# vgl-hub/kreeq

Hardware: AMD Instinct MI355X
Metric: distinct+total k-mers/sec at k=21 (count path) (higher is better)
Workload: dtype u64

## Files before the change

kreeq_amd/csrc/kq_kernels.h:

```cpp
#pragma once

#include <hip/hip_runtime.h>

#include <type_traits>

#include "../../include/kreeq_amd.h"
#include "kq_device.h"
#include "kq_partition.h"

using namespace kq;


__global__ __launch_bounds__(TILE_THREADS) void k_count_direct(TableView t, const uint8_t* __restrict__ ab,
                                                                uint64_t lead, uint64_t len, int k, EmitRange er, PartCfg filt,
                                                                const uint16_t* __restrict__ pinv ) {
    uint32_t n_new = 0;
    uint64_t n_kmers = 0;
    scan_tiles(ab, lead, len, k, [&](uint64_t pos, uint64_t fw, uint64_t rv, uint32_t prev, uint32_t next) {
        if (pos < er.lo || pos >= er.hi) return;
        const bool is_fw = fw < rv;
        const uint64_t key = is_fw ? fw : rv;
        if (filt.filt_lo != 0 || filt.filt_hi != filt.map_count) {
            const uint32_t m = map_index(key, filt.map_count, filt.map_mask);
            if (m < filt.filt_lo || m >= filt.filt_hi) return;
// ... 206 lines not shown
        tile_lane_scan_all(s_codes[half], s_inv[half], lo_valid, tile, k, er, [&](int i, bool valid, uint64_t fw, uint64_t rv, uint32_t prev, uint32_t next) {
            const bool is_fw = fw < rv;
            const uint64_t key = is_fw ? fw : rv;
            const uint64_t h = table_hash(key, (uint32_t)k);
            const uint32_t b = valid ? p1_bin_of<BINMODE>(cfg, key, h) : NB;
            if (b != NB) atomicAdd(&s_hist[b], 1u);
            if (TOP8) { s_buf[i * TILE_THREADS + lane] = top8_rec(h, edge_idx6_any(is_fw, prev, next)); s_bin[i * TILE_THREADS + lane] = (uint16_t)b; }
            else s_buf[half * MS_TILE + i * TILE_THREADS + lane] = narrow_word(narrow_main(h), narrow_aux(h, edge_idx6_any(is_fw, prev, next)), b);
        }, lane);
        __syncthreads();
        const uint32_t cnt = bin_owner ? s_hist[tid] : 0u;
        uint32_t incl = cnt;
        if (bin_owner) {
#pragma unroll
            for (int o = 1; o < 64; o <<= 1) { const uint32_t n = __shfl_up(incl, o, 64); if ((tid & 63) >= o) incl += n; }
            if ((tid & 63) == 63) s_wave[tid >> 6] = incl;
        }
        uint64_t w[16];
        uint32_t wb[TOP8 ? 16 : 1];
#pragma unroll
        for (int it = 0; it < 16; ++it) { w[it] = s_buf[half * MS_TILE + it * TILE_THREADS + lane]; if (TOP8) wb[it] = s_bin[it * TILE_THREADS + lane]; }
        __syncthreads();
        if (bin_owner) {
            uint32_t excl = incl - cnt;
            for (int v = 0; v < (tid >> 6); ++v) excl += s_wave[v];
            s_loff[tid] = excl;
            if (tid == (int)NB - 1) s_loff[NB] = excl + cnt;
            s_hist[tid] = excl;
            s_grel[tid] = gabs - excl;
            gabs += cnt;
        }
        __syncthreads();
        uint32_t pl[16];
#pragma unroll
        for (int it = 0; it < 16; ++it) { const uint32_t b = TOP8 ? wb[TOP8 ? it : 0] : narrow_word_bin(w[it]); pl[it] = b != NB ? atomicAdd(&s_hist[b], 1u) : ~0u; }
#pragma unroll
        for (int it = 0; it < 16; ++it) if (pl[it] != ~0u) { s_buf[pl[it]] = w[it]; if (TOP8) s_bin[pl[it]] = (uint16_t)wb[TOP8 ? it : 0]; }
        __syncthreads();
        const uint32_t total = s_loff[NB];
        uint64_t cv[16];
        uint32_t cg[16];
#pragma unroll
        for (int it = 0; it < 16; ++it) cv[it] = s_buf[tid + it * THREADS];
#pragma unroll
        for (int it = 0; it < 16; ++it) cg[it] = s_grel[(uint32_t)(tid + it * THREADS) < total ? (TOP8 ? (uint32_t)s_bin[TOP8 ? tid + it * THREADS : 0] : narrow_word_bin(cv[it])) : 0u] + (tid + it * THREADS);
        if (bin_owner) s_hist[tid] = 0;
        landed(nxt.x); landed(nxt.y); landed(nxt.z); landed(nxt.w);
#pragma unroll
        for (int it = 0; it < 16; ++it) {
            if ((uint32_t)(tid + it * THREADS) < total) {
                if (TOP8) reinterpret_cast<uint64_t*>(recs)[cg[it]] = cv[it];
                else { recs[cg[it]] = (uint32_t)cv[it]; recs_aux[cg[it]] = (uint8_t)(cv[it] >> 48); }
            }
        }
    }
}

__global__ __launch_bounds__(1024) void k_lv_units(const unsigned long long* __restrict__ seg_off, const unsigned long long* __restrict__ seg_hi, LevelCfg lv,
                                                   unsigned long long* __restrict__ unit_base) {
    __shared__ unsigned long long s_part[1024];
    const uint32_t tid = threadIdx.x, per = (lv.n_seg + 1023) / 1024;
    const uint32_t lo = min(tid * per, lv.n_seg), hi = min(lo + per, lv.n_seg);
    unsigned long long sum = 0;
    for (uint32_t b = lo; b < hi; ++b) sum += (seg_hi[b] - seg_off[b] + P2_UNIT - 1) / P2_UNIT;
    s_part[tid] = sum;
    __syncthreads();
    if (tid < 64) {
        unsigned long long loc[16], tot = 0;
#pragma unroll
        for (int j = 0; j < 16; ++j) { loc[j] = s_part[tid * 16 + j]; tot += loc[j]; }
        unsigned long long incl = tot;
#pragma unroll
        for (int o = 1; o < 64; o <<= 1) { unsigned long long nn = __shfl_up(incl, o, 64); if ((int)tid >= o) incl += nn; }
        unsigned long long run = incl - tot;
#pragma unroll
        for (int j = 0; j < 16; ++j) { s_part[tid * 16 + j] = run; run += loc[j]; }
        if (tid == 63) unit_base[lv.n_seg] = incl;
    }
    __syncthreads();
    unsigned long long run = s_part[tid];
    for (uint32_t b = lo; b < hi; ++b) { unit_base[b] = run; run += (seg_hi[b] - seg_off[b] + P2_UNIT - 1) / P2_UNIT; }
}
__device__ __forceinline__ uint32_t seg_of_unit(const unsigned long long* unit_base, uint32_t n_seg, uint64_t u) {
    uint32_t lo = 0, hi = n_seg;
    while (hi - lo > 1) { uint32_t mid = (lo + hi) >> 1; if (unit_base[mid] <= u) lo = mid; else hi = mid; }
    return lo;
}
template <int FMT>
__global__ __launch_bounds__(MS_THREADS) void k_lv_hist(const uint64_t* __restrict__ recs, const uint8_t* __restrict__ , LevelCfg lv,
                                                        const unsigned long long* __restrict__ seg_off, const unsigned long long* __restrict__ seg_hi,
                                                        const unsigned long long* __restrict__ unit_base, uint32_t* __restrict__ m2) {
    __shared__ uint32_t s_hist[NB_MAX];
    const uint64_t n_units = unit_base[lv.n_seg];
    for (uint64_t u = blockIdx.x; u < n_units; u += gridDim.x) {
        const uint32_t b_in = seg_of_unit(unit_base, lv.n_seg, u);
        const uint32_t b = lv.spb > 1 ? b_in / lv.spb : b_in;
        const uint64_t lo = seg_off[b_in] + (u - unit_base[b_in]) * P2_UNIT;
        const uint64_t hi = lo + P2_UNIT < seg_hi[b_in] ? lo + P2_UNIT : seg_hi[b_in];
        for (uint32_t i = threadIdx.x; i < lv.nb; i += MS_THREADS) s_hist[i] = 0;
        __syncthreads();
        const uint64_t last = hi - 1;
        if (FMT == FMT_NARROW) {
            const uint4* v4 = reinterpret_cast<const uint4*>(recs);
            const uint64_t q0 = lo >> 2, q1 = (hi + 3) >> 2;
            for (uint64_t qb = q0; qb < q1; qb += 4ull * MS_THREADS) {
                uint4 q[4];
// ... 1237 lines not shown
```

kreeq_amd/csrc/kreeq_amd.hip:

```cpp
#include <hip/hip_runtime.h>
#include <hipcub/hipcub.hpp>

#include <algorithm>
#include <cstdarg>
#include <cstdio>
#include <cstdlib>
#include <cstring>
#include <mutex>
#include <new>
#include <numeric>
#include <string>
#include <thread>
#include <type_traits>
#include <vector>

#include "../../include/kreeq_amd.h"
#include "kq_device.h"
#include "kq_partition.h"

using namespace kq;

#include "kq_kernels.h"
#include "kq_fastx.h"

// ... 577 lines not shown
    HIPC(hipStreamSynchronize(h->stream));
    std::string out;
    for (size_t i = 1; i < h->marks.size(); ++i) {
        float ms = 0;
        HIPC(hipEventElapsedTime(&ms, h->marks[i - 1].second, h->marks[i].second));
        char tmp[96];
        snprintf(tmp, sizeof tmp, "%s%s=%.4f", out.empty() ? "" : ";", h->marks[i].first, ms);
        out += tmp;
    }
    if (out.size() + 1 > cap) return fail(KQ_ERR_CAPACITY, "profile buffer too small: need %zu", out.size() + 1);
    memcpy(buf, out.c_str(), out.size() + 1);
    return KQ_OK;
}
void* kq_get_stream(kq_handle* h) { return h ? (void*)h->stream : nullptr; }
int kq_sync(kq_handle* h) {
    if (!h) return fail(KQ_ERR_INVALID, "null handle");
    HIPC(hipSetDevice(h->device));
    HIPC(hipStreamSynchronize(h->stream));
    const int rc = check_errors(h);
    if (h->fx_bad) return fail(KQ_ERR_INVALID, "malformed %s text was submitted for counting and skipped (kq_clear resets this)", h->fx_bad == KQ_FASTX_FASTQ ? "FASTQ" : "FASTA");
    return rc;
}
int kq_flush(kq_handle* h) {
    if (!h) return fail(KQ_ERR_INVALID, "null handle");
    HIPC(hipSetDevice(h->device));
    return flush_pending(h);
}
int kq_get_info(kq_handle* h, kq_info* out) {
    if (!h || !out) return fail(KQ_ERR_INVALID, "null argument");
    HIPC(hipSetDevice(h->device));
    int rc = read_state(h);
    if (rc) return rc;
    out->kmers_counted = h->st_host->kmers_added;
    out->slots_used = h->st_host->slots_used;
    out->slots_total = h->n_slots();
    out->hc_used = h->st_host->hc_used;
    out->hc_total = h->hc_cap;
    out->table_bytes = h->n_slots() * sizeof(Slot) + h->hc_cap * sizeof(HcSlot);
    out->table_passes = h->table_passes;
    return KQ_OK;
}

struct PartPlan {
    PartCfg cfg;
    bool two_level;
    int fmt;
    uint64_t n_max, R;
    uint32_t g1;
    uint64_t m1_n, m2_n, sums_n, groups_n;
    uint64_t *recs1, *recs2;
    uint8_t *aux1, *aux2;
    unsigned long long *m1, *seg_off, *unit_base, *group_base, *sums, *total, *hot;
    uint32_t* m2;
};
static void plan_cfg(const kq_handle* h, PartCfg* cfg, bool allow_narrow = false) {
    cfg->n_regions = h->n_regions;
    uint32_t g = 1;
    while (((cfg->n_regions + (1ull << g) - 1) >> g) > 512 && g < 10) ++g;
    while (((cfg->n_regions + (1ull << g) - 1) >> g) >= (uint64_t)NB_MAX) ++g;
    cfg->g_shift = cfg->n_regions < (uint64_t)NB_MAX ? 0 : g;
    cfg->n_coarse = (uint32_t)((cfg->n_regions + (1ull << cfg->g_shift) - 1) >> cfg->g_shift);
    cfg->mode = 0; cfg->map_count = (uint32_t)h->map_count;
    cfg->map_mask = (h->map_count & (h->map_count - 1)) == 0 ? (uint32_t)h->map_count - 1 : 0;
    cfg->filt_lo = 0; cfg->filt_hi = (uint32_t)h->map_count;
    cfg->raw_out = 0;
    cfg->narrow = 0; cfg->sub_bits = 0; cfg->owner_sub = 0; cfg->n_rng = 0; cfg->win_lo = 0; cfg->win_hi = 1u << NARROW_CBITS;
    if (allow_narrow && (h->k <= (int)NARROW_MAX_K || h->k > PART_MAX_K) && cfg->n_regions >= (uint64_t)NB_MAX && cfg->n_regions % (1u << NARROW_CBITS) == 0) {
        const uint64_t rps = cfg->n_regions >> NARROW_CBITS;
        uint32_t sb = 0;
        if (rps >= h->mid_rps) {
            const uint64_t target_nb = std::max<uint64_t>(1, std::min<uint64_t>(256, h->mid_rps / 8));
            while ((rps >> sb) > target_nb && sb < SUB_BITS_MAX && rps % (2ull << sb) == 0) ++sb;
        }
        if ((rps >> sb) < (uint64_t)NB_MAX && (sb > 0 || rps < (uint64_t)NB_MAX)) { cfg->narrow = 1; cfg->sub_bits = sb; }
    }
    if (cfg->narrow) { cfg->n_coarse = 1u << NARROW_CBITS; if (cfg->g_shift == 0) cfg->g_shift = 1; }
}
static int plan_alloc(kq_handle* h, PartPlan* p, uint64_t n_max, uint64_t n_tiles, uint32_t p1_bins, bool allow_narrow = false,
                      uint64_t min_segs = 0 ) {
    if (h->test_fail_plan) { h->test_fail_plan = false; return fail(KQ_ERR_NOMEM, "partition scratch allocation failed (injected by KQ_OPT_TEST_FAIL_PLAN)"); }
    if (n_max >= (1ull << 32) - 16) return fail(KQ_ERR_INVALID, "a partition pass handles fewer than 2^32 records (got %llu): slice the input", (unsigned long long)n_max);
    plan_cfg(h, &p->cfg, allow_narrow);
    n_max = (n_max + 7) & ~7ull;
    p->two_level = p->cfg.g_shift != 0;
    p->fmt = !p->cfg.narrow ? FMT_PACK8 : h->k > PART_MAX_K ? FMT_TOP8 : FMT_NARROW;
    p->n_max = n_max; p->R = p->cfg.n_regions;
    p->g1 = (uint32_t)std::max<uint64_t>(1, std::min<uint64_t>(n_tiles, (uint64_t)h->n_cu * (p1_bins < 512 ? 18 : 12)));
    p->m1_n = (uint64_t)p1_bins * p->g1 * P1_F;
    const uint64_t nb_max = std::max<uint64_t>(std::max<uint64_t>(1ull << p->cfg.g_shift, p->cfg.n_coarse), p->cfg.narrow ? (p->cfg.n_regions >> NARROW_CBITS) >> p->cfg.sub_bits : 0);
    const uint64_t seg_max = std::max<uint64_t>(min_segs, p->cfg.narrow ? ((uint64_t)1 << NARROW_CBITS) << p->cfg.sub_bits : (uint64_t)NB_MAX);
    p->m2_n = (n_max / P2_UNIT + seg_max + 2) * nb_max;
    p->groups_n = std::max<uint64_t>(std::max<uint64_t>(p->R, (uint64_t)p->cfg.n_coarse << p->cfg.g_shift), min_segs) + 2;
    p->sums_n = std::max(p->m1_n, p->groups_n) / SCAN_CHUNK + 2;
    const uint64_t aux_words = (n_max + 7) / 8 + 1;
    const uint64_t rec_words = p->fmt == FMT_NARROW ? n_max / 2 + 2 : n_max;
    const bool split2 = (rec_words + aux_words) * 8 >= ((size_t)512 << 20);
    if (split2) { int rc2 = scr_ensure(h->part2, (size_t)(rec_words + aux_words) * 8, h->device); if (rc2) return rc2; }
    const size_t words = (size_t)((split2 ? 1 : 2) * (rec_words + aux_words) + p->m1_n + 2 * (seg_max + 2) + p->groups_n + p->sums_n + 4 + (p->R + 2) + (p->m2_n + 1) / 2);
    int rc = ensure_buf(&h->part, &h->part_bytes, words * 8);
    if (rc) return rc;
    p->recs1 = (uint64_t*)h->part;
    p->aux1 = (uint8_t*)(p->recs1 + rec_words);
    uint64_t* rest = (uint64_t*)(p->aux1 + aux_words * 8);
    if (split2) { p->recs2 = (uint64_t*)h->part2.p; p->aux2 = (uint8_t*)(p->recs2 + rec_words); }
    else { p->recs2 = rest; p->aux2 = (uint8_t*)(p->recs2 + rec_words); rest = (uint64_t*)(p->aux2 + aux_words * 8); }
    p->m1 = (unsigned long long*)rest;
    p->seg_off = p->m1 + p->m1_n;
    p->unit_base = p->seg_off + seg_max + 2;
    p->group_base = p->unit_base + seg_max + 2;
    p->sums = p->group_base + p->groups_n;
    p->total = p->sums + p->sums_n;
    p->hot = p->total + 4;
    p->m2 = (uint32_t*)(p->hot + p->R + 2);
    return KQ_OK;
}
static void scan_u64(kq_handle* h, unsigned long long* a, uint64_t n, unsigned long long* sums_scratch, unsigned long long* total) {
    if (n <= 2 * SCAN_CHUNK) {
        hipLaunchKernelGGL(k_exclusive_scan, dim3(1), dim3(1024), 0, h->stream, a, n, total);
        return;
    }
    const uint64_t chunks = (n + SCAN_CHUNK - 1) / SCAN_CHUNK;
    hipLaunchKernelGGL(k_scan_sums, dim3((unsigned)chunks), dim3(1024), 0, h->stream, a, n, sums_scratch);
    hipLaunchKernelGGL(k_exclusive_scan, dim3(1), dim3(1024), 0, h->stream, sums_scratch, chunks, total);
    hipLaunchKernelGGL(k_scan_apply, dim3((unsigned)chunks), dim3(1024), 0, h->stream, a, n, sums_scratch);
}
static void mark(kq_handle* h, const char* name) {
    if (!h->profile) return;
    hipEvent_t e;
    if (hipEventCreate(&e) != hipSuccess) return;
    (void)hipEventRecord(e, h->stream);
    h->marks.emplace_back(name, e);
}
static void marks_reset(kq_handle* h) {
    for (auto& m : h->marks) (void)hipEventDestroy(m.second);
    h->marks.clear();
}

static void run_p1(kq_handle* h, PartPlan* p, const PartCfg& cfg, const uint8_t* ab, uint64_t lead, uint64_t len, EmitRange er, uint64_t* out,
                   uint8_t* out_aux, int aux_fmt, const uint16_t* pinv = nullptr ) {
    const bool plain = cfg.mode == 0 && cfg.filt_lo == 0 && cfg.filt_hi == cfg.map_count;
    const bool owner_plain = cfg.mode == 1 && cfg.map_mask != 0 && cfg.filt_lo == 0 && cfg.filt_hi == cfg.map_count;
    const bool narrow_filt = cfg.mode == 0 && cfg.narrow && !plain && cfg.map_mask != 0 && h->k <= (int)NARROW_MAX_K;
    const bool narrow_win = plain && cfg.narrow && h->k <= (int)NARROW_MAX_K && (cfg.win_lo != 0 || cfg.win_hi != (1u << NARROW_CBITS));
    const int binmode = owner_plain ? 3 : narrow_filt ? 4 : narrow_win ? 6 : !plain ? 0 : cfg.narrow ? 2 : 1;
    auto cached_hist = [&](const kq_handle::HistKey& key, size_t bytes, auto launch) -> kq_handle::HistEntry* {
        for (auto& e : h->hist_cache) if (e.key == key) return &e;
        if (h->hist_cache_bytes + bytes > ((size_t)4 << 30)) return nullptr;
        unsigned long long* buf = nullptr;
        if (hipMalloc((void**)&buf, bytes) != hipSuccess) { (void)hipGetLastError(); return nullptr; }
        launch(buf);
        h->hist_cache.push_back(kq_handle::HistEntry{key, buf, bytes});
        h->hist_cache_bytes += bytes;
        return &h->hist_cache.back();
    };
    bool have_hist = false;
    const size_t row = (size_t)p->g1 * sizeof(unsigned long long), block = row << NARROW_CBITS;
    if (narrow_filt && h->map_passes > 1 && P1_F == 1 && !h->hist_cache_off) {
        const uint32_t n = (uint32_t)h->map_passes, per = cfg.map_count / n, rr = cfg.filt_lo / per;
        if (cfg.filt_lo == rr * per && cfg.filt_hi == (rr + 1) * per) {
            const auto* ent = cached_hist({ab, pinv, lead, len, er.lo, er.hi, p->g1, n, h->k}, n * block, [&](unsigned long long* buf) {
                PartCfg all = cfg;
                all.n_rng = n; all.n_coarse = n << NARROW_CBITS;
                if (h->k == 21) hipLaunchKernelGGL((k_p1_hist<5, 21>), dim3(p->g1), dim3(TILE_THREADS), 0, h->stream, ab, lead, len, h->k, all, er, p->g1, buf, pinv);
                else hipLaunchKernelGGL((k_p1_hist<5, 0>), dim3(p->g1), dim3(TILE_THREADS), 0, h->stream, ab, lead, len, h->k, all, er, p->g1, buf, pinv);
            });
            if (ent) {
                (void)hipMemcpyAsync(p->m1, (const char*)ent->m1_all + rr * block, block, hipMemcpyDeviceToDevice, h->stream);
                have_hist = true;
            }
        }
    }
    if (narrow_win && h->map_passes > 1 && P1_F == 1 && !h->hist_cache_off) {
        const auto* ent = cached_hist({ab, pinv, lead, len, er.lo, er.hi, p->g1, 0xB0C4E7u, h->k}, block, [&](unsigned long long* buf) {
            PartCfg all = cfg;
            all.win_lo = 0; all.win_hi = 1u << NARROW_CBITS;
            if (h->k == 21) hipLaunchKernelGGL((k_p1_hist<2, 21>), dim3(p->g1), dim3(TILE_THREADS), 0, h->stream, ab, lead, len, h->k, all, er, p->g1, buf, pinv);
            else hipLaunchKernelGGL((k_p1_hist<2, 0>), dim3(p->g1), dim3(TILE_THREADS), 0, h->stream, ab, lead, len, h->k, all, er, p->g1, buf, pinv);
        });
        if (ent) {
            (void)hipMemcpyAsync(p->m1, ent->m1_all, block, hipMemcpyDeviceToDevice, h->stream);
            if (cfg.win_lo) (void)hipMemsetAsync(p->m1, 0, (size_t)cfg.win_lo * row, h->stream);
            if (cfg.win_hi < (1u << NARROW_CBITS)) (void)hipMemsetAsync((char*)p->m1 + (size_t)cfg.win_hi * row, 0, (size_t)((1u << NARROW_CBITS) - cfg.win_hi) * row, h->stream);
            have_hist = true;
        }
    }
#define KQ_P1H(B, K) hipLaunchKernelGGL((k_p1_hist<B, K>), dim3(p->g1 * P1_F), dim3(TILE_THREADS), 0, h->stream, ab, lead, len, h->k, cfg, er, p->g1, p->m1, pinv)
    if (have_hist) { }
    else if (binmode == 6) { if (h->k == 21) KQ_P1H(6, 21); else KQ_P1H(6, 0); }
    else if (binmode == 2) { if (h->k == 21) KQ_P1H(2, 21); else KQ_P1H(2, 0); }
    else if (binmode == 1) { if (h->k == 31) KQ_P1H(1, 31); else KQ_P1H(1, 0); }
    else if (binmode == 3) { if (h->k == 21) KQ_P1H(3, 21); else KQ_P1H(3, 0); }
    else if (binmode == 4) { if (h->k == 21) KQ_P1H(4, 21); else KQ_P1H(4, 0); }
    else KQ_P1H(0, 0);
#undef KQ_P1H
    scan_u64(h, p->m1, (uint64_t)cfg.n_coarse * p->g1 * P1_F, p->sums, p->total);
    hipLaunchKernelGGL(k_p1_offsets, dim3((cfg.n_coarse + 256) / 256), dim3(256), 0, h->stream, p->m1, p->total, cfg, p->g1, p->seg_off);
    mark(h, "k_p1_hist+scan");
    const bool small = cfg.n_coarse < 512;
#define KQ_P1S(W, N, B, K) hipLaunchKernelGGL((k_p1_scatter<W, N, B, K>), dim3(p->g1), dim3(TILE_THREADS), 0, h->stream, ab, lead, len, h->k, cfg, er, p->m1, out, out_aux, aux_fmt, pinv)
#define KQ_P1T(B, K) do { if (h->kernel_set & 1) KQ_P1S(FMT_TOP8, 512, B, K); else \
        hipLaunchKernelGGL((k_p1_scatter_s<B, K, 1, true>), dim3(p->g1), dim3(TILE_THREADS), 0, h->stream, ab, lead, len, h->k, cfg, er, p->m1, (uint32_t*)out, out_aux, pinv); } while (0)
    if (cfg.narrow && h->k > PART_MAX_K) { if (plain && h->k == 31) KQ_P1T(2, 31); else if (plain) KQ_P1T(2, 0); else KQ_P1T(0, 0); }
#define KQ_P1N(B, K, T) do { if (h->kernel_set & 1) KQ_P1S(FMT_NARROW, 512, B, K); else \
        hipLaunchKernelGGL((k_p1_scatter_s<B, K, T>), dim3(p->g1), dim3(TILE_THREADS * T), 0, h->stream, ab, lead, len, h->k, cfg, er, p->m1, (uint32_t*)out, out_aux, pinv); } while (0)
    else if (narrow_filt)  { if (h->k == 21) KQ_P1N(4, 21, 1); else KQ_P1N(4, 0, 1); }
    else if (narrow_win)   { if (h->k == 21) KQ_P1N(6, 21, 1); else KQ_P1N(6, 0, 1); }
    else if (cfg.narrow)   { if (plain && h->k == 21) KQ_P1N(2, 21, KQ_P1S_TPR); else if (plain) KQ_P1N(2, 0, KQ_P1S_TPR); else KQ_P1N(0, 0, 1); }
    else if (out_aux && plain && h->k == 31) { if (small) KQ_P1S(FMT_WIDE, 512, 1, 31); else KQ_P1S(FMT_WIDE, NB_MAX, 1, 31); }
    else if (out_aux) { if (small) KQ_P1S(FMT_WIDE, 512, 0, 0); else KQ_P1S(FMT_WIDE, NB_MAX, 0, 0); }
    else if (owner_plain && !out_aux && small) { if (h->k == 21) KQ_P1S(FMT_PACK8, 512, 3, 21); else KQ_P1S(FMT_PACK8, 512, 3, 0); }
    else if (plain)   { if (small) KQ_P1S(FMT_PACK8, 512, 1, 0); else KQ_P1S(FMT_PACK8, NB_MAX, 1, 0); }
    else              { if (small) KQ_P1S(FMT_PACK8, 512, 0, 0); else KQ_P1S(FMT_PACK8, NB_MAX, 0, 0); }
#undef KQ_P1S
#undef KQ_P1N
#undef KQ_P1T
    mark(h, "k_p1_scatter");
}
static void run_level(kq_handle* h, PartPlan* p, const LevelCfg& lv, const uint64_t* in, const uint8_t* in_aux, uint64_t* out, uint8_t* out_aux,
                      unsigned long long* gb = nullptr ,
                      const unsigned long long* seg_hi = nullptr ) {
    if (!gb) gb = p->group_base;
    if (!seg_hi) seg_hi = p->seg_off + 1;
    LevelCfg lvr = lv;
    lvr.rep_shift = 0;
    while (lvr.rep_shift < 6 && (((uint64_t)lv.nb + 1) << (lvr.rep_shift + 1)) <= 512) ++lvr.rep_shift;
    const LevelCfg& lv_ = lvr;
    const int fmt = lv.narrow == 2 ? FMT_TOP8 : lv.narrow ? FMT_NARROW : in_aux != nullptr ? FMT_WIDE : FMT_PACK8;
    const uint64_t groups = (uint64_t)(lv.n_seg / lv.spb) * lv.nb;
    hipLaunchKernelGGL(k_lv_units, dim3(1), dim3(1024), 0, h->stream, p->seg_off, seg_hi, lv_, p->unit_base);
    const unsigned unit_grid = (unsigned)std::min<uint64_t>(p->n_max / P2_UNIT + lv.n_seg + 1, 1u << 30);
    if (fmt == FMT_TOP8) hipLaunchKernelGGL(k_lv_hist<FMT_TOP8>, dim3(unit_grid), dim3(MS_THREADS), 0, h->stream, in, in_aux, lv_, p->seg_off, seg_hi, p->unit_base, p->m2);
    else if (fmt == FMT_NARROW) hipLaunchKernelGGL(k_lv_hist<FMT_NARROW>, dim3(unit_grid), dim3(MS_THREADS), 0, h->stream, in, in_aux, lv_, p->seg_off, seg_hi, p->unit_base, p->m2);
    else if (fmt == FMT_WIDE) hipLaunchKernelGGL(k_lv_hist<FMT_WIDE>, dim3(unit_grid), dim3(MS_THREADS), 0, h->stream, in, in_aux, lv_, p->seg_off, seg_hi, p->unit_base, p->m2);
    else hipLaunchKernelGGL(k_lv_hist<FMT_PACK8>, dim3(unit_grid), dim3(MS_THREADS), 0, h->stream, in, in_aux, lv_, p->seg_off, seg_hi, p->unit_base, p->m2);
    if (p->n_max / P2_UNIT + 1 <= 8 * (uint64_t)(lv.n_seg / lv.spb))
        hipLaunchKernelGGL(k_lv_offsets_thread, dim3((unsigned)((groups + 255) / 256)), dim3(256), 0, h->stream, p->m2, lv_, p->unit_base, gb);
    else
        hipLaunchKernelGGL(k_lv_offsets, dim3((unsigned)((groups * 64 + 255) / 256)), dim3(256), 0, h->stream, p->m2, lv_, p->unit_base, gb);
    (void)hipMemsetAsync(gb + groups, 0, 8, h->stream);
    scan_u64(h, gb, groups + 1, p->sums, p->total + 1);
    mark(h, "k_lv_hist+offsets+scan");
    const bool small = lv.nb < 512;
#define KQ_LVS(W, N) hipLaunchKernelGGL((k_lv_scatter<W, N>), dim3(unit_grid), dim3(LV_THREADS), 0, h->stream, in, in_aux, lv_, \
                                        p->seg_off, seg_hi, p->unit_base, p->m2, gb, out, out_aux)
    if (lv.top8)              { KQ_LVS(FMT_PACK8_TO_NARROW, 512); }
    else if (fmt == FMT_TOP8) { if (small) KQ_LVS(FMT_TOP8, 512); else KQ_LVS(FMT_TOP8, NB_MAX); }
#define KQ_LVN(T) hipLaunchKernelGGL((k_lv_scatter_s<T>), dim3(unit_grid), dim3(LV_THREADS), 0, h->stream, (const uint32_t*)in, in_aux, lv_, \
                                      p->seg_off, seg_hi, p->unit_base, p->m2, gb, (uint32_t*)out, out_aux)
    else if (fmt == FMT_NARROW && small && lv.rstart && !(h->kernel_set & 4)) { KQ_LVN(true); }
    else if (fmt == FMT_NARROW && small && !lv.rstart && (h->kernel_set & 2)) { KQ_LVN(false); }
#undef KQ_LVN
    else if (fmt == FMT_NARROW && lv.rstart) { if (small) KQ_LVS(FMT_NARROW_TO_TIGHT, 512); else KQ_LVS(FMT_NARROW_TO_TIGHT, NB_MAX); }
    else if (fmt == FMT_NARROW) { if (small) KQ_LVS(FMT_NARROW, 512); else KQ_LVS(FMT_NARROW, NB_MAX); }
    else if (fmt == FMT_WIDE) { if (small) KQ_LVS(FMT_WIDE, 512); else KQ_LVS(FMT_WIDE, NB_MAX); }
    else                      { if (small) KQ_LVS(FMT_PACK8, 512); else KQ_LVS(FMT_PACK8, NB_MAX); }
#undef KQ_LVS
    mark(h, "k_lv_scatter");
}
static LevelCfg level_coarse_to_regions(const PartCfg& cfg) {
    LevelCfg lv; lv.n_regions = cfg.n_regions; lv.n_seg = cfg.n_coarse; lv.nb = 1u << cfg.g_shift; lv.seg_shift = cfg.g_shift; lv.out_shift = 0; lv.in_raw = 0; lv.k = 0; lv.narrow = 0; lv.top8 = 0;
    lv.nr_shift = lv.nr_rps = lv.nr_sub = lv.nr_inv = 0; lv.nr_div = 1;
    lv.nr_mid = 0; lv.nr_fshift = 24; lv.nr_fmask = 0xFFFFFFu; lv.nr_f24 = 0;
    lv.spb = 1;
    return lv;
}
static LevelCfg level_narrow(const PartCfg& cfg, uint32_t sub_bits = 0, bool middle = false, bool top8_records = false) {
    LevelCfg lv; lv.n_regions = cfg.n_regions;
// ... 119 lines not shown
        KQ_HOT(FMT_NARROW); } while (0)
    if (fmt == FMT_TIGHT)       { if (h->k == 21) KQ_Q4(21, true); else KQ_Q4(0, true); }
    else if (fmt == FMT_NARROW) { if (h->k == 21) KQ_Q4(21, false); else KQ_Q4(0, false); }
    else if (fmt == FMT_TOP8) KQ_P3(FMT_TOP8);
    else if (fmt == FMT_WIDE) KQ_P3(FMT_WIDE);
    else KQ_P3(FMT_PACK8);
#undef KQ_Q4
#undef KQ_P3
#undef KQ_HOT
    h->n_pend = 0; h->arena_used = 0; h->pend_records = 0;
    ++h->table_passes;
    h->slots_dirty = false;
    h->table_empty = false;
    mark(h, "k_count_regions");
    HIPC(hipGetLastError());
    return KQ_OK;
}

static bool part_table_ok(const kq_handle* h, bool narrow_possible) {
    if (h->n_regions <= (1ull << 20)) return true;
    if (!narrow_possible) return false;
    PartCfg c; plan_cfg(h, &c, true);
    return c.narrow != 0;
}
static void run_narrow_levels(kq_handle* h, PartPlan* p, const uint64_t** sorted, const uint8_t** sorted_aux, const P3Set* dst, bool tight) {
    const uint32_t sb = p->cfg.sub_bits;
    const bool t8 = p->fmt == FMT_TOP8;
    uint8_t* a1 = t8 ? nullptr : p->aux1;
    uint8_t* a2 = t8 ? nullptr : p->aux2;
    uint64_t* fin = dst ? const_cast<uint64_t*>(dst->recs) : (sb == 0 ? p->recs2 : p->recs1);
    uint8_t* fin_aux = (t8 || tight) ? nullptr : dst ? const_cast<uint8_t*>(dst->aux) : (sb == 0 ? a2 : a1);
    unsigned long long* fin_base = dst ? const_cast<unsigned long long*>(dst->base) : p->group_base;
    LevelCfg last = level_narrow(p->cfg, sb, false, t8);
    if (tight) last.rstart = h->rstart;
    if (sb == 0) {
        run_level(h, p, last, p->recs1, a1, fin, fin_aux, fin_base);
    } else {
        run_level(h, p, level_narrow(p->cfg, sb, true, t8), p->recs1, a1, p->recs2, a2);
        (void)hipMemcpyAsync(p->seg_off, p->group_base, (size_t)(((1u << NARROW_CBITS) << sb) + 1) * 8, hipMemcpyDeviceToDevice, h->stream);
        run_level(h, p, last, p->recs2, a2, fin, fin_aux, fin_base);
    }
    *sorted = fin; *sorted_aux = fin_aux;
}

static int pend_or_apply(kq_handle* h, const P3Set& set, int fmt, int aux_fmt, bool in_arena) {
    int rc = pend_add(h, set, fmt, aux_fmt);
    if (rc) return rc;
    return in_arena ? KQ_OK : flush_pending(h);
}

static int count_partitioned(kq_handle* h, const uint8_t* ab, uint64_t lead, uint64_t len, EmitRange er, const uint16_t* pinv = nullptr) {
    PartPlan p;
    PartCfg c0; plan_cfg(h, &c0, true);
    int rc = plan_alloc(h, &p, len, n_tiles_of(lead, len), c0.n_coarse, true);
    if (rc) return rc;
    if (h->k > PART_MAX_K && p.fmt != FMT_TOP8) p.fmt = FMT_WIDE;
    const bool has_aux = p.fmt == FMT_WIDE || p.fmt == FMT_NARROW;
    uint8_t* a1 = has_aux ? p.aux1 : nullptr;
    uint8_t* a2 = has_aux ? p.aux2 : nullptr;
    p.cfg.filt_lo = h->filt_lo; p.cfg.filt_hi = h->filt_hi;
    if (h->windowed) { p.cfg.win_lo = h->win_lo; p.cfg.win_hi = h->win_hi; }
    const bool leveled = p.fmt == FMT_NARROW || p.fmt == FMT_TOP8 || p.two_level;
    P3Set set; bool in_arena = false;
    const bool tight = tight_ok(h, p);
    const int set_fmt = tight ? FMT_TIGHT : p.fmt;
    const bool filtered = p.cfg.filt_lo != 0 || p.cfg.filt_hi != p.cfg.map_count || h->windowed;
    if (leveled && !filtered) { rc = arena_take(h, p.n_max, set_fmt, p.R, &set, &in_arena); if (rc) return rc; }
    marks_reset(h);
    mark(h, "start");
    run_p1(h, &p, p.cfg, ab, lead, len, er, p.recs1, a1, AUX_IDX6, pinv);
    if (leveled && filtered) {
        unsigned long long n_recs = 0;
        HIPC(hipMemcpyAsync(&n_recs, p.total, sizeof n_recs, hipMemcpyDeviceToHost, h->stream));
        HIPC(hipStreamSynchronize(h->stream));
        rc = arena_take(h, std::min<uint64_t>(p.n_max, ((uint64_t)n_recs + 15) & ~7ull), set_fmt, p.R, &set, &in_arena); if (rc) return rc;
    }
    if (p.fmt == FMT_NARROW || p.fmt == FMT_TOP8) {
        const uint64_t* sorted; const uint8_t* sorted_aux;
        run_narrow_levels(h, &p, &sorted, &sorted_aux, in_arena ? &set : nullptr, tight);
        if (!in_arena) set = P3Set{sorted, sorted_aux, p.group_base, p.n_max};
    } else if (p.two_level) {
        if (in_arena) run_level(h, &p, level_coarse_to_regions(p.cfg), p.recs1, a1, const_cast<uint64_t*>(set.recs), const_cast<uint8_t*>(set.aux), const_cast<unsigned long long*>(set.base));
        else { run_level(h, &p, level_coarse_to_regions(p.cfg), p.recs1, a1, p.recs2, a2); set = P3Set{p.recs2, a2, p.group_base, p.n_max}; }
    } else {
        set = P3Set{p.recs1, a1, p.seg_off, p.n_max};
    }
    HIPC(hipGetLastError());
    return pend_or_apply(h, set, set_fmt, tight ? AUX_TIGHT : AUX_IDX6, in_arena);
}
static int count_partitioned_records(kq_handle* h, const uint64_t* d_recs, const uint8_t* d_aux, int aux_fmt, uint64_t n, bool raw) {
    PartPlan p;
    int rc = plan_alloc(h, &p, n, 0, 1, !d_aux && !raw);
    if (rc) return rc;
    P3Set set; bool in_arena = false;
    if (p.fmt == FMT_NARROW) {
        const bool tight = tight_ok(h, p);
        rc = arena_take(h, p.n_max, tight ? FMT_TIGHT : p.fmt, p.R, &set, &in_arena); if (rc) return rc;
        hipLaunchKernelGGL(k_set2, dim3(1), dim3(1), 0, h->stream, p.seg_off, 0ull, (unsigned long long)n);
        LevelCfg first = level_flat_to_coarse(p.cfg);
        first.top8 = 1; first.nb = 1u << NARROW_CBITS;
        run_level(h, &p, first, d_recs, nullptr, p.recs1, p.aux1);
        HIPC(hipMemcpyAsync(p.seg_off, p.group_base, (size_t)((1u << NARROW_CBITS) + 1) * 8, hipMemcpyDeviceToDevice, h->stream));
        const uint64_t* sorted; const uint8_t* sorted_aux;
        run_narrow_levels(h, &p, &sorted, &sorted_aux, in_arena ? &set : nullptr, tight);
        if (!in_arena) set = P3Set{sorted, sorted_aux, p.group_base, p.n_max};
        HIPC(hipGetLastError());
        return pend_or_apply(h, set, tight ? FMT_TIGHT : FMT_NARROW, tight ? AUX_TIGHT : AUX_IDX6, in_arena);
// ... 594 lines not shown
    hipLaunchKernelGGL(k_summary, dim3(grid_for(h, h->n_slots(), 1024)), dim3(256), 0, h->stream, h->view(), d_so, d_small, d_big);
    r->small.resize(HIST_SMALL);
    HIPC(hipMemcpyAsync(&r->so, d_so, sizeof(SummaryOut), hipMemcpyDeviceToHost, h->stream));
    HIPC(hipMemcpyAsync(r->small.data(), d_small, HIST_SMALL * sizeof(unsigned long long), hipMemcpyDeviceToHost, h->stream));
    HIPC(hipStreamSynchronize(h->stream));
    if (r->so.n_big > big_cap) return fail(KQ_ERR_HIP, "summary: high-coverage list overflow");
    r->big.resize(r->so.n_big);
    if (r->so.n_big) {
        HIPC(hipMemcpyAsync(r->big.data(), d_big, r->so.n_big * sizeof(uint32_t), hipMemcpyDeviceToHost, h->stream));
        HIPC(hipStreamSynchronize(h->stream));
    }
    return KQ_OK;
}
int kq_summary(kq_handle* h, kq_stats* out) {
    if (!h || !out) return fail(KQ_ERR_INVALID, "null argument");
    HIPC(hipSetDevice(h->device));
    int rc = check_errors(h);
    if (rc) return rc;
    SummaryHost r;
    rc = run_summary(h, &r);
    if (rc) return rc;
    out->total = r.so.total; out->unique = r.so.uniq; out->distinct = r.so.distinct; out->edges = r.so.edges;
    const uint64_t space = h->k < 32 ? (1ull << (2 * h->k)) : 0ull;
    out->missing = space - out->distinct;
    return KQ_OK;
}
int kq_histogram(kq_handle* h, uint64_t* cov, uint64_t* cnt, uint64_t cap, uint64_t* n_out) {
    if (!h || !n_out) return fail(KQ_ERR_INVALID, "null argument");
    HIPC(hipSetDevice(h->device));
    int rc = check_errors(h);
    if (rc) return rc;
    SummaryHost r;
    rc = run_summary(h, &r);
    if (rc) return rc;
    std::vector<std::pair<uint64_t, uint64_t>> hist;
    for (uint32_t c = 0; c < HIST_SMALL; ++c) if (r.small[c]) hist.emplace_back(c, r.small[c]);
    std::sort(r.big.begin(), r.big.end());
    for (size_t i = 0; i < r.big.size();) {
        size_t j = i; while (j < r.big.size() && r.big[j] == r.big[i]) ++j;
        hist.emplace_back(r.big[i], j - i);
        i = j;
    }
    *n_out = hist.size();
    if (!cov || !cnt) return KQ_OK;
    if (hist.size() > cap) return fail(KQ_ERR_CAPACITY, "histogram buffer too small: need %zu", hist.size());
    for (size_t i = 0; i < hist.size(); ++i) { cov[i] = hist[i].first; cnt[i] = hist[i].second; }
    return KQ_OK;
}

static int lookup_partitioned(kq_handle* h, const uint8_t* ab, uint64_t lead, uint64_t len, EmitRange er, uint32_t cov_cutoff,
                              uint32_t map_lo, uint32_t map_hi, unsigned long long* d_counters) {
    PartPlan p;
    PartCfg c0; plan_cfg(h, &c0, true);
    int rc = plan_alloc(h, &p, len, n_tiles_of(lead, len), c0.n_coarse, true);
    if (rc) return rc;
    if (h->k > PART_MAX_K && p.fmt != FMT_TOP8) p.fmt = FMT_WIDE;
    const bool has_aux = p.fmt == FMT_WIDE || p.fmt == FMT_NARROW;
    uint8_t* a1 = has_aux ? p.aux1 : nullptr;
    uint8_t* a2 = has_aux ? p.aux2 : nullptr;
    p.cfg.filt_lo = map_lo; p.cfg.filt_hi = map_hi;
    run_p1(h, &p, p.cfg, ab, lead, len, er, p.recs1, a1, AUX_IDX6);
    const uint64_t* sorted = p.recs1; const uint8_t* sorted_aux = a1; const unsigned long long* base = p.seg_off;
    if (p.fmt == FMT_NARROW || p.fmt == FMT_TOP8) {
        run_narrow_levels(h, &p, &sorted, &sorted_aux);
        base = p.group_base;
    } else if (p.two_level) {
        run_level(h, &p, level_coarse_to_regions(p.cfg), p.recs1, a1, p.recs2, a2);
        sorted = p.recs2; sorted_aux = a2; base = p.group_base;
    }
    const uint32_t rps = (p.fmt == FMT_NARROW || p.fmt == FMT_TOP8) ? (uint32_t)(p.R >> NARROW_CBITS) : 1u;
    const dim3 grid((unsigned)std::min<uint64_t>(p.R, 1u << 30)), block(P3_THREADS);
#define KQ_LK(F) hipLaunchKernelGGL((k_lookup_regions<F>), grid, block, 0, h->stream, h->view(), sorted, sorted_aux, base, rps, cov_cutoff, d_counters)
    if (p.fmt == FMT_NARROW) KQ_LK(FMT_NARROW); else if (p.fmt == FMT_TOP8) KQ_LK(FMT_TOP8); else if (p.fmt == FMT_WIDE) KQ_LK(FMT_WIDE); else KQ_LK(FMT_PACK8);
#undef KQ_LK
    HIPC(hipGetLastError());
    return KQ_OK;
}

int kq_lookup_sequence_dev(kq_handle* h, const char* d_bases, uint64_t len, uint32_t cov_cutoff, uint16_t map_lo, uint16_t map_hi,
                           kq_dbgbase* d_per_base, uint64_t* d_counters) {
    if (!h || !d_counters || (!d_bases && len)) return fail(KQ_ERR_INVALID, "null argument");
    if (map_lo > map_hi || map_hi > h->map_count) return fail(KQ_ERR_INVALID, "map range [%u,%u) outside [0,%d]", map_lo, map_hi, h->map_count);
    HIPC(hipSetDevice(h->device));
    if (len < (uint64_t)h->k) return KQ_OK;
    const uint8_t* ab; uint64_t lead;
    aligned_view(d_bases, &ab, &lead);
    const uint32_t map_mask = (h->map_count & (h->map_count - 1)) == 0 ? (uint32_t)h->map_count - 1 : 0;
    { int frc = flush_pending(h); if (frc) return frc; }
    materialize(h);
    const uint64_t kmers = len - h->k + 1;
    if (!d_per_base && h->lookup_path != 1 && part_table_ok(h, true) &&
        (h->lookup_path == 2 || (kmers >= (1u << 20) && (double)h->n_slots() * sizeof(Slot) <= 64.0 * (double)std::min<uint64_t>(kmers, h->slice_kmers)))) {
        for (uint64_t a = 0; a < kmers; a += h->slice_kmers) {
            const uint64_t b = std::min(kmers, a + h->slice_kmers);
            const uint64_t sub_off = a ? a - 1 : 0;
            const uint64_t sub_len = std::min(len, b + h->k) - sub_off;
            const uint8_t* sab; uint64_t slead;
            aligned_view(d_bases + sub_off, &sab, &slead);
            int rc = lookup_partitioned(h, sab, slead, sub_len, EmitRange{a - sub_off, b - sub_off}, cov_cutoff, map_lo, map_hi, (unsigned long long*)d_counters);
            if (rc) return rc;
        }
        return KQ_OK;
    }
    const dim3 grid(grid_for(h, n_tiles_of(lead, len), 1, 32));
    if (d_per_base) hipLaunchKernelGGL(k_lookup<true>, grid, dim3(TILE_THREADS), 0, h->stream, h->view(), ab, lead, len, h->k, (uint32_t)h->map_count,
                                       map_mask, (uint32_t)map_lo, (uint32_t)map_hi, cov_cutoff, d_per_base, (unsigned long long*)d_counters);
    else hipLaunchKernelGGL(k_lookup<false>, grid, dim3(TILE_THREADS), 0, h->stream, h->view(), ab, lead, len, h->k, (uint32_t)h->map_count,
// ... 206 lines not shown
```

Measured before the change: 51.53 billion.

## Add filtered narrow P1 scatter kernel that batches several tiles per block

Adds a new phase-1 scatter kernel for the filtered narrow-format path. It scans up to T tiles per block and compacts the surviving k-mers into a shared-memory queue, spilling the overflow to a per-block global buffer. It then hashes, bins and scatters the queue in full MS_TILE rounds. The goal is to avoid running a full histogram and scatter round for every tile when the map filter keeps only a fraction of k-mers. In exchange it adds spill scratch memory, extra global traffic for the overflow, and a new launch-selection path.

```diff
diff --git a/kreeq_amd/csrc/kq_kernels.h b/kreeq_amd/csrc/kq_kernels.h
--- a/kreeq_amd/csrc/kq_kernels.h
+++ b/kreeq_amd/csrc/kq_kernels.h
@@ -282,6 +282,113 @@
                 if (TOP8) reinterpret_cast<uint64_t*>(recs)[cg[it]] = cv[it];
                 else { recs[cg[it]] = (uint32_t)cv[it]; recs_aux[cg[it]] = (uint8_t)(cv[it] >> 48); }
             }
+        }
+    }
+}
+
+constexpr uint32_t P1F_QCAP = MS_TILE;
+constexpr uint32_t P1F_MAX_T = 4;
+__host__ __device__ constexpr uint32_t p1f_spill_words(uint32_t t) { return t * TILE_STARTS - P1F_QCAP; }
+template <int KC, int T>
+__global__ __launch_bounds__(TILE_THREADS, 4) void k_p1_scatter_f(const uint8_t* __restrict__ ab, uint64_t lead, uint64_t len, int k_arg,
+                                                             PartCfg cfg, EmitRange er, const unsigned long long* __restrict__ m1,
+                                                             uint32_t* __restrict__ recs, uint8_t* __restrict__ recs_aux,
+                                                             const uint16_t* __restrict__ pinv ,
+                                                             uint64_t* spill_all ) {
+    constexpr uint32_t NB = 1u << NARROW_CBITS;
+    static_assert(NB == TILE_THREADS && MS_TILE == TILE_THREADS * 16 && P1F_QCAP == MS_TILE && T >= 2 && T <= (int)P1F_MAX_T && T * TILE_STARTS > (int)P1F_QCAP, "thread b owns bin b; round 0 is the queue");
+    __shared__ uint32_t s_codes[2][TILE_THREADS];
+    __shared__ uint32_t s_inv[2][TILE_THREADS];
+    __shared__ uint64_t s_q[P1F_QCAP];
+    __shared__ uint32_t s_hist[NB], s_grel[NB], s_wave[TILE_THREADS / 64], s_tail;
+    const int k = KC ? KC : k_arg;
+    const int tid = threadIdx.x;
+    const int64_t lo_valid = (int64_t)lead, hi_valid = (int64_t)(lead + len);
+    const uint64_t n_tiles = n_tiles_of(lead, len);
+    uint64_t* const spill = spill_all + (uint64_t)blockIdx.x * p1f_spill_words(T);
+    uint32_t gabs = (uint32_t)m1[(uint64_t)tid * gridDim.x * P1_F + (uint64_t)blockIdx.x * P1_F];
+    s_hist[tid] = 0;
+    if (tid == 0) s_tail = 0;
+    uint4 nxt = tile_fetch(ab, lo_valid, hi_valid, blockIdx.x, pinv);
+    landed(nxt.x); landed(nxt.y); landed(nxt.z); landed(nxt.w);
+    for (uint64_t tile0 = blockIdx.x; tile0 < n_tiles; tile0 += (uint64_t)gridDim.x * T) {
+#pragma unroll 1
+        for (int g = 0; g < T; ++g) {
+            const uint64_t tile = tile0 + (uint64_t)g * gridDim.x;
+            if (tile >= n_tiles) break;
+            tile_store(nxt, lo_valid, hi_valid, tile, s_codes[g & 1], s_inv[g & 1], pinv != nullptr);
+            if (tile + gridDim.x < n_tiles) nxt = tile_fetch(ab, lo_valid, hi_valid, tile + gridDim.x, pinv);
+            tile_lane_scan_all(s_codes[g & 1], s_inv[g & 1], lo_valid, tile, k, er, [&](int, bool valid, uint64_t fw, uint64_t rv, uint32_t prev, uint32_t next) {
+                const bool is_fw = fw < rv;
+                const uint64_t key = is_fw ? fw : rv;
+                const bool keep = valid && ((uint32_t)key & cfg.map_mask) - cfg.filt_lo < cfg.filt_hi - cfg.filt_lo;
+                const uint64_t bal = __ballot(keep);
+                if (bal) {
+                    uint32_t base = 0;
+                    if ((tid & 63) == 0) base = atomicAdd(&s_tail, (uint32_t)__popcll(bal));
+                    base = __builtin_amdgcn_readfirstlane(base);
+                    if (keep) {
+                        const uint32_t pos = base + __builtin_amdgcn_mbcnt_hi((uint32_t)(bal >> 32), __builtin_amdgcn_mbcnt_lo((uint32_t)bal, 0u));
+                        const uint32_t hi = (uint32_t)(key >> 32) | ((uint32_t)is_fw << 10) | (prev << 11) | (next << 14);
+                        const uint64_t q = (uint64_t)(uint32_t)key | ((uint64_t)hi << 32);
+                        if (pos < P1F_QCAP) s_q[pos] = q; else spill[pos - P1F_QCAP] = q;
+                    }
+                }
+            });
+        }
+        __syncthreads();
+        const uint32_t n = s_tail;
+        for (uint32_t r0 = 0; r0 < n; r0 += MS_TILE) {
+            const uint32_t m = n - r0 < (uint32_t)MS_TILE ? n - r0 : (uint32_t)MS_TILE;
+            uint64_t w[16];
+#pragma unroll
+            for (int it = 0; it < 16; ++it) {
+                const uint32_t j = (uint32_t)(tid + it * TILE_THREADS);
+                                w[it] = j < m ? (r0 == 0 ? s_q[j] : spill[r0 - P1F_QCAP + j]) : 0ull;
+            }
+#pragma unroll
+            for (int it = 0; it < 16; ++it) {
+                const uint32_t hi = (uint32_t)(w[it] >> 32);
+                const uint64_t key = (w[it] & 0xFFFFFFFFull) | ((uint64_t)(hi & 0x3FFu) << 32);
+                const uint64_t h = table_hash(key, (uint32_t)k);
+                const uint32_t b = (uint32_t)(tid + it * TILE_THREADS) < m ? (uint32_t)(h >> (64 - NARROW_CBITS)) : NB;
+                if (b != NB) atomicAdd(&s_hist[b], 1u);
+                w[it] = narrow_word(narrow_main(h), narrow_aux(h, edge_idx6_any((hi >> 10) & 1u, (hi >> 11) & 7u, (hi >> 14) & 7u)), b);
+                landed(w[it]);
+            }
+            __syncthreads();
+            const uint32_t cnt = s_hist[tid];
+            uint32_t incl = cnt;
+#pragma unroll
+            for (int o = 1; o < 64; o <<= 1) { const uint32_t v = __shfl_up(incl, o, 64); if ((tid & 63) >= o) incl += v; }
+            if ((tid & 63) == 63) s_wave[tid >> 6] = incl;
+            if (tid == 0) s_tail = 0;
+            __syncthreads();
+            uint32_t excl = incl - cnt;
+            for (int v = 0; v < (tid >> 6); ++v) excl += s_wave[v];
+            s_hist[tid] = excl;
+            s_grel[tid] = gabs - excl;
+            gabs += cnt;
+            __syncthreads();
+            uint32_t pl[16];
+#pragma unroll
+            for (int it = 0; it < 16; ++it) { const uint32_t b = narrow_word_bin(w[it]); pl[it] = b != NB ? atomicAdd(&s_hist[b], 1u) : ~0u; }
+#pragma unroll
+            for (int it = 0; it < 16; ++it) if (pl[it] != ~0u) s_q[pl[it]] = w[it];
+            __syncthreads();
+            uint64_t cv[16];
+            uint32_t cg[16];
+#pragma unroll
+            for (int it = 0; it < 16; ++it) cv[it] = s_q[tid + it * TILE_THREADS];
+#pragma unroll
+            for (int it = 0; it < 16; ++it) cg[it] = s_grel[(uint32_t)(tid + it * TILE_THREADS) < m ? narrow_word_bin(cv[it]) : 0u] + (tid + it * TILE_THREADS);
+            s_hist[tid] = 0;
+            landed(nxt.x); landed(nxt.y); landed(nxt.z); landed(nxt.w);
+#pragma unroll
+            for (int it = 0; it < 16; ++it) {
+                if ((uint32_t)(tid + it * TILE_THREADS) < m) { recs[cg[it]] = (uint32_t)cv[it]; recs_aux[cg[it]] = (uint8_t)(cv[it] >> 48); }
+            }
+            if (r0 + MS_TILE < n) __syncthreads();
         }
     }
 }
diff --git a/kreeq_amd/csrc/kreeq_amd.hip b/kreeq_amd/csrc/kreeq_amd.hip
--- a/kreeq_amd/csrc/kreeq_amd.hip
+++ b/kreeq_amd/csrc/kreeq_amd.hip
@@ -653,7 +653,13 @@
     uint8_t *aux1, *aux2;
     unsigned long long *m1, *seg_off, *unit_base, *group_base, *sums, *total, *hot;
     uint32_t* m2;
+    uint32_t p1f_t;
+    uint64_t* p1f_spill;
 };
+static uint32_t p1f_tiles(uint32_t map_count, uint32_t filt_lo, uint32_t filt_hi) {
+    if (filt_hi <= filt_lo) return 1;
+    return std::max<uint32_t>(1, std::min<uint32_t>(P1F_MAX_T, map_count / (filt_hi - filt_lo)));
+}
 static void plan_cfg(const kq_handle* h, PartCfg* cfg, bool allow_narrow = false) {
     cfg->n_regions = h->n_regions;
     uint32_t g = 1;
@@ -678,7 +684,8 @@
     if (cfg->narrow) { cfg->n_coarse = 1u << NARROW_CBITS; if (cfg->g_shift == 0) cfg->g_shift = 1; }
 }
 static int plan_alloc(kq_handle* h, PartPlan* p, uint64_t n_max, uint64_t n_tiles, uint32_t p1_bins, bool allow_narrow = false,
-                      uint64_t min_segs = 0 ) {
+                      uint64_t min_segs = 0 ,
+                      uint32_t filt_lo = 0, uint32_t filt_hi = 0 ) {
     if (h->test_fail_plan) { h->test_fail_plan = false; return fail(KQ_ERR_NOMEM, "partition scratch allocation failed (injected by KQ_OPT_TEST_FAIL_PLAN)"); }
     if (n_max >= (1ull << 32) - 16) return fail(KQ_ERR_INVALID, "a partition pass handles fewer than 2^32 records (got %llu): slice the input", (unsigned long long)n_max);
     plan_cfg(h, &p->cfg, allow_narrow);
@@ -697,7 +704,9 @@
     const uint64_t rec_words = p->fmt == FMT_NARROW ? n_max / 2 + 2 : n_max;
     const bool split2 = (rec_words + aux_words) * 8 >= ((size_t)512 << 20);
     if (split2) { int rc2 = scr_ensure(h->part2, (size_t)(rec_words + aux_words) * 8, h->device); if (rc2) return rc2; }
-    const size_t words = (size_t)((split2 ? 1 : 2) * (rec_words + aux_words) + p->m1_n + 2 * (seg_max + 2) + p->groups_n + p->sums_n + 4 + (p->R + 2) + (p->m2_n + 1) / 2);
+    p->p1f_t = (p->fmt == FMT_NARROW && n_tiles && p->cfg.map_mask != 0 && filt_hi != 0) ? p1f_tiles(p->cfg.map_count, filt_lo, filt_hi) : 1;
+    const uint64_t spill_words = p->p1f_t > 1 ? (uint64_t)p->g1 * p1f_spill_words(p->p1f_t) : 0;
+    const size_t words = (size_t)((split2 ? 1 : 2) * (rec_words + aux_words) + p->m1_n + 2 * (seg_max + 2) + p->groups_n + p->sums_n + 4 + (p->R + 2) + (p->m2_n + 1) / 2 + 1 + spill_words);
     int rc = ensure_buf(&h->part, &h->part_bytes, words * 8);
     if (rc) return rc;
     p->recs1 = (uint64_t*)h->part;
@@ -713,6 +722,7 @@
     p->total = p->sums + p->sums_n;
     p->hot = p->total + 4;
     p->m2 = (uint32_t*)(p->hot + p->R + 2);
+    p->p1f_spill = spill_words ? (uint64_t*)p->m2 + (p->m2_n + 1) / 2 + 1 : nullptr;
     return KQ_OK;
 }
 static void scan_u64(kq_handle* h, unsigned long long* a, uint64_t n, unsigned long long* sums_scratch, unsigned long long* total) {
@@ -802,9 +812,14 @@
 #define KQ_P1T(B, K) do { if (h->kernel_set & 1) KQ_P1S(FMT_TOP8, 512, B, K); else \
         hipLaunchKernelGGL((k_p1_scatter_s<B, K, 1, true>), dim3(p->g1), dim3(TILE_THREADS), 0, h->stream, ab, lead, len, h->k, cfg, er, p->m1, (uint32_t*)out, out_aux, pinv); } while (0)
     if (cfg.narrow && h->k > PART_MAX_K) { if (plain && h->k == 31) KQ_P1T(2, 31); else if (plain) KQ_P1T(2, 0); else KQ_P1T(0, 0); }
-#define KQ_P1N(B, K, T) do { if (h->kernel_set & 1) KQ_P1S(FMT_NARROW, 512, B, K); else \
-        hipLaunchKernelGGL((k_p1_scatter_s<B, K, T>), dim3(p->g1), dim3(TILE_THREADS * T), 0, h->stream, ab, lead, len, h->k, cfg, er, p->m1, (uint32_t*)out, out_aux, pinv); } while (0)
-    else if (narrow_filt)  { if (h->k == 21) KQ_P1N(4, 21, 1); else KQ_P1N(4, 0, 1); }
+#define KQ_P1N_S(B, K, T) hipLaunchKernelGGL((k_p1_scatter_s<B, K, T>), dim3(p->g1), dim3(TILE_THREADS * T), 0, h->stream, ab, lead, len, h->k, cfg, er, p->m1, (uint32_t*)out, out_aux, pinv)
+#define KQ_P1N(B, K, T) do { if (h->kernel_set & 1) KQ_P1S(FMT_NARROW, 512, B, K); else KQ_P1N_S(B, K, T); } while (0)
+#define KQ_P1F(K, T) hipLaunchKernelGGL((k_p1_scatter_f<K, T>), dim3(p->g1), dim3(TILE_THREADS), 0, h->stream, ab, lead, len, h->k, cfg, er, p->m1, (uint32_t*)out, out_aux, pinv, p->p1f_spill)
+    else if (narrow_filt)  {
+        const uint32_t t = (h->kernel_set & 1) ? 1 : std::min(p1f_tiles(cfg.map_count, cfg.filt_lo, cfg.filt_hi), p->p1f_t);
+        if (h->k == 21) { if (t == 4) KQ_P1F(21, 4); else if (t == 3) KQ_P1F(21, 3); else if (t == 2) KQ_P1F(21, 2); else KQ_P1N_S(4, 21, 1); }
+        else            { if (t == 4) KQ_P1F(0, 4);  else if (t == 3) KQ_P1F(0, 3);  else if (t == 2) KQ_P1F(0, 2);  else KQ_P1N_S(4, 0, 1); }
+    }
     else if (narrow_win)   { if (h->k == 21) KQ_P1N(6, 21, 1); else KQ_P1N(6, 0, 1); }
     else if (cfg.narrow)   { if (plain && h->k == 21) KQ_P1N(2, 21, KQ_P1S_TPR); else if (plain) KQ_P1N(2, 0, KQ_P1S_TPR); else KQ_P1N(0, 0, 1); }
     else if (out_aux && plain && h->k == 31) { if (small) KQ_P1S(FMT_WIDE, 512, 1, 31); else KQ_P1S(FMT_WIDE, NB_MAX, 1, 31); }
@@ -814,6 +829,8 @@
     else              { if (small) KQ_P1S(FMT_PACK8, 512, 0, 0); else KQ_P1S(FMT_PACK8, NB_MAX, 0, 0); }
 #undef KQ_P1S
 #undef KQ_P1N
+#undef KQ_P1N_S
+#undef KQ_P1F
 #undef KQ_P1T
     mark(h, "k_p1_scatter");
 }
@@ -1039,7 +1056,7 @@
 static int count_partitioned(kq_handle* h, const uint8_t* ab, uint64_t lead, uint64_t len, EmitRange er, const uint16_t* pinv = nullptr) {
     PartPlan p;
     PartCfg c0; plan_cfg(h, &c0, true);
-    int rc = plan_alloc(h, &p, len, n_tiles_of(lead, len), c0.n_coarse, true);
+    int rc = plan_alloc(h, &p, len, n_tiles_of(lead, len), c0.n_coarse, true, 0, h->filt_lo, h->filt_hi);
     if (rc) return rc;
     if (h->k > PART_MAX_K && p.fmt != FMT_TOP8) p.fmt = FMT_WIDE;
     const bool has_aux = p.fmt == FMT_WIDE || p.fmt == FMT_NARROW;
@@ -1740,7 +1757,7 @@
                               uint32_t map_lo, uint32_t map_hi, unsigned long long* d_counters) {
     PartPlan p;
     PartCfg c0; plan_cfg(h, &c0, true);
-    int rc = plan_alloc(h, &p, len, n_tiles_of(lead, len), c0.n_coarse, true);
+    int rc = plan_alloc(h, &p, len, n_tiles_of(lead, len), c0.n_coarse, true, 0, map_lo, map_hi);
     if (rc) return rc;
     if (h->k > PART_MAX_K && p.fmt != FMT_TOP8) p.fmt = FMT_WIDE;
     const bool has_aux = p.fmt == FMT_WIDE || p.fmt == FMT_NARROW;
```

Result: slower. 50.63 billion (-1.7%).
